# AI-Unicamp/interspeech_ser

Measured on AMD Instinct MI355X. Metric: utterances/sec (10 s @16 kHz) WavLM-large embed extract, higher is better.
Workload: dtype bf16; 1 GPU; microsoft/wavlm-large embed extract, batch=16 x 10 s @16 kHz per GPU, all 25 hidden states to HBM, mode=bf16; a counted step = 8 such batches (128 utterances per GPU), 2 in flight at a time; batch=16, batches_in_flight=2, frames_per_utt=499, parallelism=utterance-sharded x1, no collective (one process)

## Files before the change

include/ser_hip.h:

```cpp
#ifndef SER_HIP_H
#define SER_HIP_H

#include <stddef.h>
#include <stdint.h>

#ifdef __cplusplus
extern "C" {
#endif

#define SER_ABI_VERSION 18

#define SER_MODE_BF16  1
#define SER_MODE_FP32X 2
#define SER_MODE_FP16  3
#define SER_MODE_FP16X 4
#define SER_MODE_FP16Q 5

#define SER_MODE_FP16M 6

#define SER_ACT_NONE 0
#define SER_ACT_GELU 1

int         ser_version(void);
const char* ser_last_error(void);
// ... 174 lines not shown
typedef struct ser_row_center_args {
    const float* x; int64_t ldx; void* out_act; int64_t ldo_act; int64_t out_plane_stride;
    float* stats; float* shift; int32_t stat_groups, mode, rows, D;
    uint32_t* out_scale; int64_t out_scale_ld;
    uint32_t* range_flag;
} ser_row_center_args;
int ser_row_center_v(const ser_row_center_args* args, void* stream);

typedef struct ser_logmel_args {
    const float* wav; const int64_t* sample_offs; const float* mel; float* out; void* work; int32_t B, n_mels;
} ser_logmel_args;

typedef struct ser_pack_act_args {
    const float* x; void* out; int64_t ldo; int64_t out_plane_stride; int32_t B, C, T, halo, mode, reserved0;
    uint32_t* range_flag;
} ser_pack_act_args;
int ser_pack_act_v(const ser_pack_act_args* args, void* stream);

typedef struct ser_wave_frames_args {
    const float* wav; const int64_t* sample_offs; const int32_t* frame_offs; int32_t B, k, stride, mode;
    void* out; int64_t out_plane_stride; void* work; int32_t total_rows;
    int32_t no_norm;
    uint32_t* range_flag;
} ser_wave_frames_args;
int ser_wave_frames_v(const ser_wave_frames_args* args, void* stream);

#define SER_RESAMPLE_TILE 1024
typedef struct ser_resample_args {
    const float* wav; const int64_t* in_offs; const int64_t* out_offs;
    const int32_t* up; const int32_t* down; const int32_t* half; const int64_t* bank_off;
    const double* bank; float* out;
    int64_t total_in, total_out, max_out;
    int32_t B, reserved0;
} ser_resample_args;
int ser_resample_v(const ser_resample_args* args, void* stream);

typedef struct ser_gn_stats_args {
    const float* wav; const int64_t* sample_offs; const int32_t* frame_offs;
    const float* w; const float* bias; const float* gamma; const float* beta;
    const void* wave_stats;
    float* scale; float* shift; float* stat_out; void* work;
    int32_t B, C, k, stride, ld, no_norm;
    float eps; int32_t reserved0;
} ser_gn_stats_args;
int ser_gn_stats_v(const ser_gn_stats_args* args, void* stream);

// ... 310 lines not shown
```

interspeech_ser_amd/_lib.py:

```python
from __future__ import annotations

import ctypes as C
import os

import torch

_HERE = os.path.dirname(os.path.abspath(__file__))
LIB_PATH = os.environ.get("SER_HIP_LIB") or os.path.join(_HERE, "lib", "libserhip.so")

MODE_BF16 = 1
MODE_FP32X = 2
MODE_FP16 = 3
MODE_FP16X = 4
MODE_FP16Q = 5
MODE_FP16M = 6
ACT_NONE = 0
ACT_GELU = 1
WS_LOGMEL = 1
WS_WAVE_FRAMES = 2
WS_GN_STATS = 3
GRU_ERR_TIMEOUT = 1
RESAMPLE_TILE = 1024
SELECT_ROWS_TILE = 8
ABI_VERSION = 18
# ... 39 lines not shown
        ("gate_x", c_void_p), ("gate_x_ld", c_i64), ("gate_x_plane_stride", c_i64),
        ("gate_stat", c_void_p), ("gate_w", c_void_p), ("gate_cb", c_void_p),
        ("gate_x_planes", C.c_int32), ("reserved1", C.c_int32), ("gate_w_plane_stride", c_i64),
        ("out_scale", c_void_p), ("out_scale_ld", c_i64),
    ]


class LayerNormArgs(C.Structure):
    _fields_ = [
        ("x", c_void_p), ("ldx", c_i64), ("g", c_void_p), ("b", c_void_p), ("eps", c_float), ("gelu", C.c_int32),
        ("out_f32", c_void_p), ("ldo_f32", c_i64), ("out_act", c_void_p), ("ldo_act", c_i64), ("out_plane_stride", c_i64),
        ("mode", C.c_int32), ("rows", C.c_int32), ("D", C.c_int32), ("reserved0", C.c_int32),
        ("range_flag", c_void_p),
    ]


class WaveFramesArgs(C.Structure):
    _fields_ = [
        ("wav", c_void_p), ("sample_offs", c_void_p), ("frame_offs", c_void_p),
        ("B", C.c_int32), ("k", C.c_int32), ("stride", C.c_int32), ("mode", C.c_int32),
        ("out", c_void_p), ("out_plane_stride", c_i64), ("work", c_void_p),
        ("total_rows", C.c_int32), ("no_norm", C.c_int32),
        ("range_flag", c_void_p),
    ]


class GnStatsArgs(C.Structure):
    _fields_ = [
        ("wav", c_void_p), ("sample_offs", c_void_p), ("frame_offs", c_void_p),
        ("w", c_void_p), ("bias", c_void_p), ("gamma", c_void_p), ("beta", c_void_p),
        ("wave_stats", c_void_p),
        ("scale", c_void_p), ("shift", c_void_p), ("stat_out", c_void_p), ("work", c_void_p),
        ("B", C.c_int32), ("C", C.c_int32), ("k", C.c_int32), ("stride", C.c_int32), ("ld", C.c_int32), ("no_norm", C.c_int32),
        ("eps", c_float), ("reserved0", C.c_int32),
    ]


class RowCenterArgs(C.Structure):
    _fields_ = [
        ("x", c_void_p), ("ldx", c_i64), ("out_act", c_void_p), ("ldo_act", c_i64), ("out_plane_stride", c_i64),
        ("stats", c_void_p), ("shift", c_void_p),
        ("stat_groups", C.c_int32), ("mode", C.c_int32), ("rows", C.c_int32), ("D", C.c_int32),
        ("out_scale", c_void_p), ("out_scale_ld", c_i64), ("range_flag", c_void_p),
    ]


# ... 369 lines not shown
```

interspeech_ser_amd/csrc/gemm.hip:

```cpp
#include "ser_common.h"
#include "launch_plan.h"
#ifndef SER_GEMM_PP
#define SER_GEMM_PP 27
#endif
#include <stdlib.h>
#include <stdio.h>
#include <utility>
#ifdef SER_GEMM_DBG
extern "C" { void* ser_gemm_dbg_ptr = nullptr; }
__device__ unsigned long long* ser_gemm_dbg_dev = nullptr;
#endif

typedef const __attribute__((address_space(1))) void* gptr_t;
typedef __attribute__((address_space(3))) void* lptr_t;

__device__ __forceinline__ const char* uniform_ptr(const void* p) {
    const uint64_t v = (uint64_t)p;
    const uint32_t lo = __builtin_amdgcn_readfirstlane((uint32_t)v), hi = __builtin_amdgcn_readfirstlane((uint32_t)(v >> 32));
    return (const char*)(((uint64_t)hi << 32) | lo);
}
template <int BYTES>
__device__ __forceinline__ void dma_lds(const void* ubase, uint32_t voff, uint32_t lds_addr) {
    static_assert(BYTES == 16 || BYTES == 4, "dwordx4 or dword");
    if constexpr (BYTES == 16)
// ... 19 lines not shown
    else static_assert(N < 0, "add a case");
}

__device__ __forceinline__ void mfma_scale8(f32x4& acc, const i32x8& a, const i32x8& b, int sa, int sb) {
    asm volatile("v_mfma_scale_f32_16x16x128_f8f6f4 %0, %1, %2, %0, %3, %4 op_sel_hi:[0,0,0]" : "+v"(acc) : "v"(a), "v"(b), "v"(sa), "v"(sb));
}
__device__ __forceinline__ void mfma_scale_drain() {
    asm volatile("s_nop 15\n\ts_nop 15\n\ts_nop 7" ::: "memory");
}

template <int WM, int WN, int TM, int TN, int BK, int ST, int MODE, bool LNEPI, int OM = MODE>
__global__ __launch_bounds__(64 * WM * WN, 2)
void ser_gemm_kernel(const ser_gemm_args p) {
    constexpr int NW = WM * WN, NT = 64 * NW;
    constexpr int BM = WM * TM * 16, BN = WN * TN * 16;
    constexpr int CH = BK / 8;
    constexpr int ROWB = BK * 2;
    constexpr int RPP = 1024 / ROWB;
    constexpr bool M16 = (MODE == SER_MODE_FP16M);
    constexpr int NPL = M16 ? 1 : mode_traits<MODE>::planes;
    constexpr int A_BYTES = BM * ROWB, W_BYTES = BN * ROWB, STAGE = NPL * (A_BYTES + W_BYTES);
    static_assert(!M16 || (BK == 64 && !LNEPI && (BM + BN) % 64 == 0), "FP16M: 64-deep K tiles, dense epilogue");
    constexpr int SCW = BM + BN;
    constexpr int LA = BM / RPP / NW, LW = BN / RPP / NW;
    constexpr int LPT = NPL * (LA + LW);
    constexpr int KS = BK / 32;
    static_assert(BM % (RPP * NW) == 0 && BN % (RPP * NW) == 0, "tile/wave mismatch");
    extern __shared__ __attribute__((aligned(16))) char lds[];

    const int tid = threadIdx.x;
    const int lane = tid & 63;
    const int wave = __builtin_amdgcn_readfirstlane(tid >> 6);
    const int wm = wave / WN, wn = wave % WN;
#ifdef SER_GEMM_DBG
    const unsigned long long dbg_e0 = __builtin_amdgcn_s_memtime();
#endif

    const int ntn = (p.N + BN - 1) / BN;
    const int ntm = (p.M + BM - 1) / BM;
    int bid = blockIdx.x;
    {
        const int nwg = ntm * ntn;
        const int q = nwg >> 3, r = nwg & 7, xcd = bid & 7;
        const int base = (xcd < r) ? xcd * (q + 1) : r * (q + 1) + (xcd - r) * q;
        bid = base + (bid >> 3);
    }
    const int mt = bid / ntn;
    const int nt = bid - mt * ntn;
    const int g = blockIdx.y;
    const int m0 = mt * BM, n0 = nt * BN;
// ... 43 lines not shown
        int i = sc_is_a ? m0 + r : n0 + r - BM;
        const int lim = sc_is_a ? p.M : p.N;
        i = i < lim ? i : lim - 1;
        sc_off = (uint32_t)i * 4u;
    }
    int i_kk = 0, i_cc = 0, i_cj = 0, i_stage = 0;
    const char* is_ua = nullptr; const char* is_uw = nullptr;
    uint32_t is_dstA = 0, is_dstW = 0;
    auto issue_begin = [&]() {
        int64_t koffA = (int64_t)i_cj * p.ldj + (int64_t)i_cc * BK;
        int64_t koffW = (int64_t)i_kk * BK;
        if constexpr (M16) {
            koffA = (int64_t)(i_kk >> 1) * BK + (i_kk & 1) * p.a_plane_stride;
            koffW = (int64_t)(i_kk >> 1) * BK + (i_kk & 1) * p.w_plane_stride;
            if (i_kk & 1) dma_lds<4>(sc_base + (int64_t)(i_kk >> 1) * sc_step, sc_off, lds0 + (uint32_t)(ST * STAGE + (LNEPI ? 0 : BM * 8) + (i_stage * SCW + sc_chunk * 64) * 4));
        }
        is_dstA = lds0 + i_stage * STAGE + wave * 1024;
        is_dstW = is_dstA + NPL * A_BYTES;
        is_ua = Atile + koffA * 2;
        is_uw = Wtile + koffW * 2;
    };
    auto issue_piece = [&](int j) {
        const int pl = j / (LA + LW), q = j % (LA + LW);
        if (q < LA) dma_lds<16>(is_ua + (int64_t)pl * p.a_plane_stride * 2, aoff[q < LA ? q : 0], is_dstA + pl * A_BYTES + q * NW * 1024);
        else dma_lds<16>(is_uw + (int64_t)pl * p.w_plane_stride * 2, woff[q >= LA ? q - LA : 0], is_dstW + pl * W_BYTES + (q - LA) * NW * 1024);
    };
    auto issue_end = [&]() {
        ++i_kk; ++i_cc;
        if (i_cc == tpc) { i_cc = 0; ++i_cj; }
        i_stage = (i_stage + 1 == ST) ? 0 : i_stage + 1;
    };
    auto issue = [&]() {
        issue_begin();
#pragma unroll
        for (int j = 0; j < LPT; ++j) issue_piece(j);
        issue_end();
    };

    f32x4 acc[TN][TM];
#pragma unroll
    for (int a = 0; a < TN; ++a)
#pragma unroll
        for (int b = 0; b < TM; ++b) acc[a][b] = (f32x4){0.f, 0.f, 0.f, 0.f};

    const int frow = lane & 15, fq = lane >> 4;
    const int fsw = (BK == 64) ? (lane & 7) : ((frow >> 1) & 3);
    int offA[KS], offW[KS];
// ... 681 lines not shown
```

interspeech_ser_amd/csrc/launch_plan.h:

```cpp
#pragma once
#include <stddef.h>
#include <stdint.h>
#include <stdio.h>
#include <stdlib.h>
#include "../../include/ser_hip.h"

int ser_fail(int code, const char* fmt, ...);

#ifdef SER_EXPERIMENTS
static inline long ser_knob(const char* name, long dflt) { const char* e = getenv(name); return e ? atol(e) : dflt; }
#else
constexpr long ser_knob(const char*, long dflt) { return dflt; }
#endif

struct gemm_tile {
    const char* name;
    int WM, WN, TM, TN, BK, ST;
    bool LNEPI, two_plane;
    constexpr int BM() const { return WM * TM * 16; }
    constexpr int BN() const { return WN * TN * 16; }
    constexpr int threads() const { return 64 * WM * WN; }
    constexpr bool dense() const { return !LNEPI && BN() >= 128; }
};
enum gemm_tile_id {
    GEMM_128x128, GEMM_256x128, GEMM_256x256,
    GEMM_128x64, GEMM_LN512, GEMM_LN512_M64, GEMM_LN512_M32,
    GEMM_X_128x128x64, GEMM_X_256x128x32, GEMM_X_256x256x32, GEMM_X_128x64x32, GEMM_X_LN128x512x32,
    GEMM_TILES
};
constexpr gemm_tile GEMM_TILE[GEMM_TILES] = {
    {"128x128",         2, 2, 4, 4, 64, 2, false, false},
    {"256x128",         4, 2, 4, 4, 64, 3, false, false},
    {"256x256",         2, 4, 8, 4, 64, 2, false, false},
    {"128x64",          4, 1, 2, 4, 64, 2, false, false},
    {"LN512",           2, 4, 4, 8, 64, 2, true,  false},
    {"LN512_M64",       1, 8, 4, 4, 64, 2, true,  false},
    {"LN512_M32",       1, 4, 2, 8, 64, 2, true,  false},
    {"X_128x128x64",    4, 2, 2, 4, 64, 2, false, true},
    {"X_256x128x32",    4, 2, 4, 4, 32, 3, false, true},
    {"X_256x256x32",    4, 2, 4, 8, 32, 2, false, true},
    {"X_128x64x32",     4, 1, 2, 4, 32, 2, false, true},
    {"X_LN128x512x32",  2, 4, 4, 8, 32, 2, true,  true},
};

struct gemm_pair { int mode, om; };
constexpr gemm_pair GEMM_PAIR[] = {
    {SER_MODE_BF16, SER_MODE_BF16},
    {SER_MODE_FP16, SER_MODE_FP16},
    {SER_MODE_FP16, SER_MODE_FP16X},
    {SER_MODE_FP16M, SER_MODE_FP16M},
    {SER_MODE_FP16M, SER_MODE_FP16X},
    {SER_MODE_FP32X, SER_MODE_FP32X},
    {SER_MODE_FP32X, SER_MODE_FP16},
    {SER_MODE_FP16X, SER_MODE_FP16X},
    {SER_MODE_FP16X, SER_MODE_FP16},
    {SER_MODE_FP16X, SER_MODE_FP16M},
};
constexpr int GEMM_PAIRS = (int)(sizeof(GEMM_PAIR) / sizeof(GEMM_PAIR[0]));
constexpr int gemm_pair_index(int mode, int om) {
    for (int i = 0; i < GEMM_PAIRS; ++i)
        if (GEMM_PAIR[i].mode == mode && GEMM_PAIR[i].om == om) return i;
    return -1;
}
constexpr bool gemm_two_plane(int mode) { return mode == SER_MODE_FP32X || mode == SER_MODE_FP16X; }
constexpr bool gemm_tile_serves(const gemm_tile& t, gemm_pair p) {
    if (t.two_plane != gemm_two_plane(p.mode)) return false;
    if (p.mode == SER_MODE_FP16M) return t.dense() && t.BK == 64;
    if (p.om == p.mode) return true;
    if (t.two_plane && p.om == SER_MODE_FP16) return !t.LNEPI;
    return t.dense();
}

struct gemm_knobs {
    int ln_bm, n64, deepk;
    long t256_min, x32_256_min, x32_sq_min, m16_sq_min, m16_256_min;
};
static inline const gemm_knobs& gemm_knobs_get() {
    static const gemm_knobs k = {
        (int)ser_knob("SER_GEMM_LN_BM", 0), (int)ser_knob("SER_GEMM_N64", 1), (int)ser_knob("SER_GEMM_DEEPK_256x128", 1),
        ser_knob("SER_GEMM_T256_MIN", 150),
        ser_knob("SER_GEMM_X32_256_MIN", 100),
        ser_knob("SER_GEMM_X32_SQ_MIN", 150), ser_knob("SER_GEMM_M16_SQ_MIN", 100), ser_knob("SER_GEMM_M16_256_MIN", 100)};
    return k;
}

#ifdef SER_EXPERIMENTS
static inline int gemm_forced_tile(const ser_gemm_args* a) {
    struct Rule { int n, k, cfg; };
    static Rule rules[8];
    static const int nrules = [] {
        const char* e = getenv("SER_GEMM_FORCE");
        int n = 0;
        while (e && *e && n < 8) {
            int a0, a1, a2, used = 0;
            if (sscanf(e, "%d:%d:%d%n", &a0, &a1, &a2, &used) != 3) break;
            rules[n++] = {a0, a1, a2};
            e += used;
            if (*e == ',') ++e;
        }
        return n;
    }();
    for (int i = 0; i < nrules; ++i)
        if (rules[i].n == a->N && rules[i].k == a->K && rules[i].cfg >= 0 && rules[i].cfg <= GEMM_256x256) return rules[i].cfg;
    return -1;
}
#endif

static inline int gemm_pick_tile(const ser_gemm_args* a) {
    const gemm_knobs& kn = gemm_knobs_get();
    const long rt256 = (a->M + 255) / 256;
    const long t256sq = rt256 * ((a->N + 255) / 256) * a->groups;
    const long t256x128 = rt256 * ((a->N + 127) / 128) * a->groups;
    if (gemm_two_plane(a->mode)) {
        if (a->ln_gamma) return GEMM_X_LN128x512x32;
        if (kn.n64 && a->N <= 64) return GEMM_X_128x64x32;
        const long sq_rounds = (t256sq + 255) / 256;
        const bool sq_full = t256sq * 100 >= sq_rounds * 256 * 85;
        if (kn.x32_sq_min > 0 && a->N >= 256 && t256sq >= kn.x32_sq_min && sq_full && a->act == SER_ACT_NONE) return GEMM_X_256x256x32;
        if (kn.x32_256_min > 0 && a->N >= 128 && t256x128 >= kn.x32_256_min) return GEMM_X_256x128x32;
        return GEMM_X_128x128x64;
    }
    if (a->mode == SER_MODE_FP16M) {
        if (a->tile_cfg == 3 || (!a->tile_cfg && a->N >= 256 && t256sq >= kn.m16_sq_min)) return GEMM_256x256;
        if (a->tile_cfg == 2 || (!a->tile_cfg && a->N >= 128 && t256x128 >= kn.m16_256_min)) return GEMM_256x128;
        return GEMM_128x128;
    }
    if (a->ln_gamma) {
        const int bm = kn.ln_bm ? kn.ln_bm : (a->M >= 200 * 128 ? 128 : (a->M >= 200 * 64 ? 64 : 32));
        return bm == 128 ? GEMM_LN512 : (bm == 64 ? GEMM_LN512_M64 : GEMM_LN512_M32);
    }
    if (a->tile_cfg > 0) return a->tile_cfg - 1;
#ifdef SER_EXPERIMENTS
    if (const int forced = gemm_forced_tile(a); forced >= 0) return forced;
#endif
    if (a->N >= 256 && t256sq >= kn.t256_min) return GEMM_256x256;
    if (kn.n64 && a->N <= 64) return GEMM_128x64;
    if (kn.deepk && a->groups == 1 && a->K >= 2048 && a->N >= 128 && a->M >= 512) return GEMM_256x128;
    return GEMM_128x128;
}

struct gemm_launch {
    int tile, pair;
    unsigned grid_x, grid_y;
    int block, lds;
};

static inline int gemm_plan(const ser_gemm_args* a, gemm_launch* out) {
    if (!a || !a->A || !a->W) return ser_fail(-1, "ser_gemm: null operand");
    if (a->M <= 0 || a->N <= 0 || a->K <= 0) return ser_fail(-2, "ser_gemm: bad shape M=%d N=%d K=%d", a->M, a->N, a->K);
    if (a->K % 64) return ser_fail(-3, "ser_gemm: K=%d must be a multiple of 64", a->K);
    if (a->kc && (a->kc % 64 || a->K % a->kc)) return ser_fail(-4, "ser_gemm: kc=%d must divide K and be a multiple of 64", a->kc);
    if (a->N % 8) return ser_fail(-5, "ser_gemm: N=%d must be a multiple of 8", a->N);
    if (gemm_pair_index(a->mode, a->mode) < 0) return ser_fail(-6, "ser_gemm: bad mode %d", a->mode);
    if (a->mode == SER_MODE_FP16M) {
        if (!a->a_scale || !a->w_scale || a->a_scale_ld < a->M || a->w_scale_ld < a->N)
            return ser_fail(-23, "ser_gemm: FP16M needs a_scale / w_scale with *_scale_ld >= the row count");
        if (a->a_rowoff || a->kc || a->groups != 1 || a->ln_gamma || (a->lda % 64))
            return ser_fail(-23, "ser_gemm: FP16M takes plain row-major operands (no row map / conv chunks / groups / LayerNorm epilogue), lda %% 64 == 0");
    }
    if (a->out_mode == SER_MODE_FP16M || (a->mode == SER_MODE_FP16M && !a->out_mode && a->out_act)) {
        if (!a->out_scale || (a->N % 64) || (a->ldo_act % 64) || a->groups != 1 || a->ln_gamma)
            return ser_fail(-24, "ser_gemm: an FP16M out_act needs out_scale, N %% 64 == 0, ldo_act %% 64 == 0, groups == 1, no LayerNorm epilogue");
    }
    if (!a->a_rowoff && (a->lda % 8)) return ser_fail(-7, "ser_gemm: lda must be a multiple of 8");
    if (a->groups < 1) return ser_fail(-8, "ser_gemm: groups=%d", a->groups);
    if (!a->out_f32 && !a->out_act) return ser_fail(-9, "ser_gemm: no output");
    if ((a->ldo_f32 % 4) || (a->ldo_act % 4) || (a->ldr % 4) || (a->c_group_stride % 4))
        return ser_fail(-10, "ser_gemm: output/residual pitches must be multiples of 4");
    if (a->ln_gamma) {
        if (!a->ln_beta) return ser_fail(-11, "ser_gemm: ln_gamma without ln_beta");
        if (a->N > 512 || a->groups != 1 || a->residual)
            return ser_fail(-12, "ser_gemm: the LayerNorm epilogue needs N <= 512, groups == 1, no residual");
    }
    if (a->ln_stats_in) {
        if (!a->ln_colsum || a->ln_groups < 2 || a->ln_groups > 32 || (a->ln_groups & 1) || a->ln_gamma)
            return ser_fail(-14, "ser_gemm: deferred LayerNorm needs ln_colsum, an even ln_groups in [2,32] and no fused-LN epilogue");
    }
    if (a->stat_out && (a->ln_gamma || a->stat_groups < a->groups * ((a->N + 63) / 64)))
        return ser_fail(-15, "ser_gemm: stat_out needs stat_groups >= groups*ceil(N/64) and no fused-LN epilogue");
    if (a->shift_out && (!a->stat_out || a->ln_gamma)) return ser_fail(-19, "ser_gemm: shift_out needs stat_out and no fused-LN epilogue");
    if (a->mean_out && !a->ln_stats_in) return ser_fail(-20, "ser_gemm: mean_out needs ln_stats_in");
    if (a->lnstat_out && !a->ln_stats_in) return ser_fail(-20, "ser_gemm: lnstat_out needs ln_stats_in");
    const int om = a->out_mode ? a->out_mode : a->mode;
    const int pair = gemm_pair_index(a->mode, om);
    if (om != a->mode && !a->ln_gamma && pair < 0)
        return ser_fail(-21, "ser_gemm: out_mode %d with mode %d (FP32X -> FP16, FP16 <-> FP16X, FP16X <-> FP16M convert)", a->out_mode, a->mode);
    if (om != a->mode && a->ln_gamma) return ser_fail(-21, "ser_gemm: out_mode %d with the LayerNorm epilogue", a->out_mode);
    if (a->col_scale_end % 4) return ser_fail(-17, "ser_gemm: col_scale_end must be a multiple of 4");
    if (a->gn_scale && (!a->gn_shift || !a->gn_row_offs || a->gn_B < 1 || a->gn_ld < a->N || (a->gn_ld % 4) || a->groups != 1 ||
                        a->ln_gamma || a->ln_stats_in))
        return ser_fail(-25, "ser_gemm: gn_scale needs gn_shift, gn_row_offs, gn_B >= 1, gn_ld >= N (multiple of 4), groups == 1, "
                             "no LayerNorm epilogue and no deferred LayerNorm");
    if ((a->ldo_act % 8) || (a->c_group_stride % 8)) return ser_fail(-18, "ser_gemm: act pitch / group stride must be multiples of 8");
    if (a->f32_col_begin < 0 || (a->f32_col_begin % 8)) return ser_fail(-16, "ser_gemm: f32_col_begin must be a non-negative multiple of 8");
    if (a->tile_cfg < 0 || a->tile_cfg > 3) return ser_fail(-13, "ser_gemm: tile_cfg=%d (0 auto, 1..3)", a->tile_cfg);

    const int tile = gemm_pick_tile(a);
    const gemm_tile& t = GEMM_TILE[tile];
    if (!gemm_tile_serves(t, GEMM_PAIR[pair])) {
        if (a->mode == SER_MODE_FP16M) return ser_fail(-22, "ser_gemm: FP16M needs a dense tile (N > 64, no LayerNorm epilogue)");
        if (a->mode == SER_MODE_FP16X) return ser_fail(-22, "ser_gemm: FP16X -> FP16M output needs a dense tile (N > 64)");
        return ser_fail(-22, "ser_gemm: FP16 -> FP16X output needs a dense tile (N > 64, no LayerNorm epilogue)");
    }
    const int BM = t.BM(), BN = t.BN();
    out->tile = tile;
    out->pair = pair;
    out->grid_x = (unsigned)(((a->M + BM - 1) / BM) * ((a->N + BN - 1) / BN));
    out->grid_y = (unsigned)a->groups;
    out->block = t.threads();
    out->lds = (gemm_two_plane(a->mode) ? 2 : 1) * t.ST * (BM + BN) * t.BK * 2 + (t.LNEPI ? 0 : BM * 8)
             + (a->mode == SER_MODE_FP16M ? t.ST * (BM + BN) * 4 : 0);
    return 0;
}

constexpr int ATTN_BKV = 64;
constexpr int ATTN_NWV = 4;

struct attn_launch {
    int dhp, mode;
    bool pre, tbl, b2d, gb, occ;
    int nbuf, bias_stride;
    size_t lds;
    int nq;
    unsigned grid;
};
constexpr int attn_qk_planes(int mode) { return (mode == SER_MODE_FP32X || mode == SER_MODE_FP16X || mode == SER_MODE_FP16Q) ? 2 : 1; }
constexpr int attn_v_planes(int mode) { return (mode == SER_MODE_FP32X || mode == SER_MODE_FP16X) ? 2 : 1; }
constexpr bool attn_form_built(int dhp, int mode, bool pre, bool tbl, bool b2d, bool gb, bool occ) {
    if (b2d) return dhp == 64 && pre && !tbl && !gb && !occ && (mode == SER_MODE_BF16 || mode == SER_MODE_FP32X || mode == SER_MODE_FP16X);
    if (gb) return dhp == 64 && pre && tbl && !occ;
    if (occ) return dhp == 64 && attn_qk_planes(mode) == 1;
    return pre || (mode != SER_MODE_FP16X && mode != SER_MODE_FP16Q);
}
// ... 64 lines not shown
```

interspeech_ser_amd/csrc/rowops.hip:

```cpp
#include "row_common.h"

__global__ __launch_bounds__(1024) void wave_norm_kernel(const float* __restrict__ wav,
                                                         const int64_t* __restrict__ offs, float* __restrict__ out) {
    __shared__ double red[16];
    __shared__ float stat[2];
    const int b = blockIdx.x;
    const int64_t s0 = offs[b], n = offs[b + 1] - s0;
    const float* x = wav + s0;
    float* y = out + s0;
    const int tid = threadIdx.x, lane = tid & 63, wv = tid >> 6;

    double acc = 0.0;
    for (int64_t i = tid; i < n; i += 1024) acc += (double)x[i];
    for (int o = 32; o > 0; o >>= 1) acc += __shfl_xor(acc, o, 64);
    if (lane == 0) red[wv] = acc;
    __syncthreads();
    if (tid == 0) {
        double t = 0.0;
        for (int i = 0; i < 16; ++i) t += red[i];
        stat[0] = (float)(t / (double)n);
    }
    __syncthreads();
    const float mean = stat[0];
    acc = 0.0;
// ... 20 lines not shown

__global__ __launch_bounds__(256) void wave_stats_kernel(const float* __restrict__ wav, const int64_t* __restrict__ offs,
                                                         double* __restrict__ part ) {
    __shared__ double red[2][4];
    const int b = blockIdx.y, chunk = blockIdx.x;
    const int64_t s0 = offs[b], n = offs[b + 1] - s0;
    const int64_t per = (n + 63) / 64;
    const int64_t lo = chunk * per, hi = (lo + per < n) ? lo + per : n;
    double a1 = 0.0, a2 = 0.0;
    for (int64_t i = lo + threadIdx.x; i < hi; i += 256) { const double x = (double)wav[s0 + i]; a1 += x; a2 += x * x; }
    for (int o = 32; o > 0; o >>= 1) { a1 += __shfl_xor(a1, o, 64); a2 += __shfl_xor(a2, o, 64); }
    if ((threadIdx.x & 63) == 0) { red[0][threadIdx.x >> 6] = a1; red[1][threadIdx.x >> 6] = a2; }
    __syncthreads();
    if (threadIdx.x == 0) {
        part[((int64_t)b * 64 + chunk) * 2] = (red[0][0] + red[0][1]) + (red[0][2] + red[0][3]);
        part[((int64_t)b * 64 + chunk) * 2 + 1] = (red[1][0] + red[1][1]) + (red[1][2] + red[1][3]);
    }
}

template <int MODE>
__global__ __launch_bounds__(256) void wave_frames_kernel(const float* __restrict__ wav, const int64_t* __restrict__ soffs,
                                                          const int32_t* __restrict__ foffs, const double* __restrict__ part,
                                                          unsigned short* __restrict__ out, int64_t plane, int k, int stride, uint32_t* __restrict__ rflag,
                                                          int no_norm) {
    __shared__ float stat[2];
    float ramax = 0.f;
    const int b = blockIdx.y, tid = threadIdx.x;
    const int64_t s0 = soffs[b], n = soffs[b + 1] - s0;
    if (tid < 64) {
        double a1 = part[((int64_t)b * 64 + tid) * 2], a2 = part[((int64_t)b * 64 + tid) * 2 + 1];
        for (int o = 32; o > 0; o >>= 1) { a1 += __shfl_xor(a1, o, 64); a2 += __shfl_xor(a2, o, 64); }
        if (tid == 0) {
            const double mean = a1 / (double)n;
            const double var = a2 / (double)n - mean * mean;
            stat[0] = (float)mean;
            stat[1] = 1.0f / sqrtf((float)(var > 0.0 ? var : 0.0) + 1e-7f);
        }
    }
    __syncthreads();
    const float mean = no_norm ? 0.f : stat[0], rstd = no_norm ? 1.f : stat[1];
    const int row_begin = foffs[b], T = foffs[b + 1] - row_begin;
    const float* x = wav + s0;
    const int c = tid & 7;
    for (int t = blockIdx.x * 32 + (tid >> 3); t < T; t += gridDim.x * 32) {
        float v[8];
#pragma unroll
        for (int i = 0; i < 8; ++i) {
            const int j = c * 8 + i;
            v[i] = (j < k) ? (x[(int64_t)t * stride + j] - mean) * rstd : 0.f;
        }
        unsigned short* dst = out + (int64_t)(row_begin + t) * 64 + c * 8;
        store_act4<MODE>(dst, plane, v[0], v[1], v[2], v[3]);
        store_act4<MODE>(dst + 4, plane, v[4], v[5], v[6], v[7]);
        if constexpr (mode_traits<MODE>::f16) {
#pragma unroll
            for (int i = 0; i < 8; ++i) ramax = range_fold(ramax, v[i]);
        }
    }
    if constexpr (mode_traits<MODE>::f16) range_report(rflag, ramax);
}

extern "C" int ser_wave_frames_v(const ser_wave_frames_args* a, void* stream) {
    if (!a) return ser_fail(-1, "ser_wave_frames: null pointer");
    const float* wav = a->wav; const int64_t* sample_offs = a->sample_offs; const int32_t* frame_offs = a->frame_offs;
    const int B = a->B, k = a->k, stride = a->stride, mode = a->mode, total_rows = a->total_rows;
    void* out = a->out; const int64_t out_plane_stride = a->out_plane_stride; void* work = a->work;
    if (!wav || !sample_offs || !frame_offs || !out || !work) return ser_fail(-1, "ser_wave_frames: null pointer");
    if (B <= 0 || k < 1 || k > 64 || stride < 1 || total_rows <= 0) return ser_fail(-2, "ser_wave_frames: bad B/k/stride/rows");
    if (mode != SER_MODE_BF16 && mode != SER_MODE_FP32X && mode != SER_MODE_FP16X) return ser_fail(-3, "ser_wave_frames: bad mode");
    hipStream_t s = (hipStream_t)stream;
    hipLaunchKernelGGL(wave_stats_kernel, dim3(64, B), dim3(256), 0, s, wav, sample_offs, (double*)work);
    int blocks = ((total_rows + B - 1) / B + 31) / 32;
    if (blocks > 1024) blocks = 1024;
    if (blocks < 1) blocks = 1;
    ser_with_mode<SER_MODE_BF16, SER_MODE_FP32X, SER_MODE_FP16X>(mode, [&](auto M) {
        hipLaunchKernelGGL(wave_frames_kernel<M()>, dim3(blocks, B), dim3(256), 0, s, wav, sample_offs, frame_offs, (const double*)work,
                           (unsigned short*)out, out_plane_stride, k, stride, a->range_flag, a->no_norm);
    });
    return ser_check_launch("ser_wave_frames");
}

extern "C" int ser_wave_frames(const float* wav, const int64_t* sample_offs, const int32_t* frame_offs, int B, int k,
                               int stride, void* out, int64_t out_plane_stride, int mode, void* work, int total_rows,
                               void* stream) {
    ser_wave_frames_args a = {};
    a.wav = wav; a.sample_offs = sample_offs; a.frame_offs = frame_offs; a.B = B; a.k = k; a.stride = stride; a.mode = mode;
    a.out = out; a.out_plane_stride = out_plane_stride; a.work = work; a.total_rows = total_rows;
    return ser_wave_frames_v(&a, stream);
}

template <int CPL, int KT, int MODE>
__global__ __launch_bounds__(256) void conv0_kernel(const float* __restrict__ x, const int64_t* __restrict__ soffs,
                                                    const int32_t* __restrict__ foffs,
                                                    const float* __restrict__ w, const float* __restrict__ bias,
                                                    const float* __restrict__ lg, const float* __restrict__ lb,
                                                    unsigned short* __restrict__ out, int64_t plane,
                                                    int k, int stride, int rpg) {
    constexpr int C = CPL * 64;
    const int lane = threadIdx.x & 63;
    const int b = blockIdx.y;
// ... 730 lines not shown
```

interspeech_ser_amd/engine.py:

```python
from __future__ import annotations

import copy
import ctypes as C
import math
from dataclasses import dataclass
from typing import Dict, List, Optional, Sequence

import numpy as np
import torch

from . import _lib
from ._lib import check, lib
from .weights import check_f16_weight
from .config import EncoderGeometry, FAMILY_DATA2VEC_AUDIO, FAMILY_ROBERTA, FAMILY_W2V_BERT, FAMILY_WAVLM, FAMILY_WHISPER

MODES = {"bf16": _lib.MODE_BF16, "fp32x": _lib.MODE_FP32X, "f16": _lib.MODE_FP16, "f16q": _lib.MODE_FP16, "f16a": _lib.MODE_FP16,
         "f16x": _lib.MODE_FP16X, "f16m": _lib.MODE_FP16M, "f16mf": _lib.MODE_FP16M}
POST_LN_MODES = ("f16x", "fp32x", "bf16")
_PLANES = {_lib.MODE_BF16: 1, _lib.MODE_FP32X: 2, _lib.MODE_FP16: 1, _lib.MODE_FP16X: 2, _lib.MODE_FP16M: 2}
_DTYPE = {_lib.MODE_BF16: torch.bfloat16, _lib.MODE_FP32X: torch.bfloat16, _lib.MODE_FP16: torch.float16,
          _lib.MODE_FP16X: torch.float16, _lib.MODE_FP16M: torch.float16}
_PRODUCTS = {_lib.MODE_BF16: 1, _lib.MODE_FP32X: 3, _lib.MODE_FP16: 1, _lib.MODE_FP16X: 3, _lib.MODE_FP16M: 2}


import os as _os
_NO_SHIFT = _os.environ.get("SER_NO_SHIFT", "0") == "1"
_STEM_F16X = _os.environ.get("SER_STEM_F16X", "1") == "1"


def _ptr(t: Optional[torch.Tensor]) -> Optional[int]:
    return None if t is None else t.data_ptr()


def _stream() -> int:
    return torch.cuda.current_stream().cuda_stream


class Sz(int):

    def __new__(cls, value: int, name: str):
        o = int.__new__(cls, value)
        o.name = name
        return o


class Tape:

    def __init__(self, capacity: int = 640):
        self.cmds = (_lib.Cmd * capacity)()
        self.n = 0
# ... 683 lines not shown
        super().__init__(geo, device, mode, post_ln=not geo.stable_layer_norm)
        if geo.family == FAMILY_WHISPER:
            raise ValueError("use WhisperEncoder for the whisper family")
        self.normalize = bool(normalize)
        self.gn_stem = geo.feat_extract_norm == "group"
        if (geo.family == FAMILY_DATA2VEC_AUDIO) != (geo.pos_conv_norm == "layer"):
            raise NotImplementedError("the LayerNorm'd positional conv stack is data2vec-audio's, and data2vec-audio has only that one")
        if geo.family == FAMILY_DATA2VEC_AUDIO:
            if self.gn_stem or not self.post_ln:
                raise NotImplementedError("data2vec-audio: the layer-norm conv stem with a post-LN encoder is the only form")
        elif self.post_ln != self.gn_stem:
            raise NotImplementedError("GroupNorm stems come with post-LN encoders and layer-norm stems with stable-LN ones")
        if not geo.feat_proj_layer_norm:
            raise NotImplementedError("feat_proj_layer_norm=False checkpoints are not supported")
        sd = state_dict
        D, C0 = geo.hidden, geo.conv_dim[0]
        if any(c != C0 for c in geo.conv_dim):
            raise NotImplementedError("conv_dim must be uniform")
        p0 = "feature_extractor.conv_layers.0"
        self.conv0_w = self._dev_f32(sd[p0 + ".conv.weight"].reshape(C0, geo.conv_kernel[0]))
        self.conv0_b = self._dev_f32(sd[p0 + ".conv.bias"]) if geo.conv_bias else None
        if geo.conv_kernel[0] > 64:
            raise NotImplementedError("conv layer 0 kernel wider than 64 taps")
        w0 = torch.zeros((C0, 64), dtype=torch.float32)
        w0[:, : geo.conv_kernel[0]] = sd[p0 + ".conv.weight"].reshape(C0, geo.conv_kernel[0]).float()
        self.conv0 = self._linear(w0, sd[p0 + ".conv.bias"] if geo.conv_bias else None, stem=True, name=p0 + ".conv.weight")
        if self.gn_stem:
            self.gn0 = self._ln_pair(sd, p0 + ".layer_norm")
            self.conv_ln = [None] * len(geo.conv_dim)
        else:
            self.conv_ln = [self._ln_pair(sd, f"feature_extractor.conv_layers.{i}.layer_norm") for i in range(len(geo.conv_dim))]
        self.convs: List[Linear] = []
        for i in range(1, len(geo.conv_dim)):
            p = f"feature_extractor.conv_layers.{i}.conv"
            w = sd[p + ".weight"].float()
            w2 = w.permute(0, 2, 1).reshape(w.shape[0], -1)
            self.convs.append(self._linear(w2, sd[p + ".bias"] if geo.conv_bias else None, stem=True, name=p + ".weight"))
        self.proj_ln = self._ln_pair(sd, "feature_projection.layer_norm")
        self.proj = self._linear(sd["feature_projection.projection.weight"], sd["feature_projection.projection.bias"], stem=True,
                                 name="feature_projection.projection.weight")
        G, k = geo.pos_conv_groups, geo.pos_conv_kernel
        Cg = D // G
        self.pos_cg, self.pos_kc = Cg, ((Cg + 63) // 64) * 64

        def pos_weight(w: torch.Tensor) -> torch.Tensor:
            wp = torch.zeros((G, Cg, k, self.pos_kc), dtype=torch.float32)
            wp[:, :, :, :Cg] = w.float().view(G, Cg, Cg, k).permute(0, 1, 3, 2)
# ... 14 lines not shown
                a = p + ".attention"
                self.layers.append(self._post_ln_layer_weights(
                    sd, a + ".q_proj", a + ".k_proj", a + ".v_proj", a + ".out_proj", p + ".layer_norm",
                    p + ".feed_forward.intermediate_dense", p + ".feed_forward.output_dense", p + ".final_layer_norm",
                    gate=self._gate_cols(sd, a) if geo.family == FAMILY_WAVLM else None))
                continue
            self.layers.append(self._layer_weights(
                sd, p, p + ".attention", p + ".layer_norm", p + ".final_layer_norm",
                p + ".feed_forward.intermediate_dense", p + ".feed_forward.output_dense",
                k_bias=True, gate=(geo.family == FAMILY_WAVLM), index=i))
        if geo.family == FAMILY_WAVLM:
            self.rel_embed = self._dev_f32(sd["encoder.layers.0.attention.rel_attn_embed.weight"])

    def _arena(self, slot: int, need: Dict[str, int]):
        arenas = self.__dict__.setdefault("_arenas", {})
        ar = arenas.get(slot)
        if ar is not None and all(ar["cap"][k] >= v for k, v in need.items()):
            return ar
        cap = {k: max(int(v), ar["cap"][k] if ar else 0) for k, v in need.items()}
        geo, dev = self.geo, self.device
        C0, D = geo.conv_dim[0], geo.hidden
        nl = len(geo.conv_dim)
        ar = dict(cap=cap)
        ar["frames"] = self._new_act(cap["rows0"], 64, stem=True)
        ar["wave_work"] = torch.empty(lib.ser_workspace_bytes(_lib.WS_WAVE_FRAMES, cap["B"], 0, 0, 0, self.stem_mode),
                                      dtype=torch.uint8, device=dev)
        ar["conv_act"] = [self._new_act(cap["rows0"], C0, stem=True), self._new_act(cap["rows1"], C0, stem=True)]
        ar["conv_rowoff"] = [torch.empty(cap["rows1"], dtype=torch.int32, device=dev) for _ in range(1, nl)]
        ar["halo_rowmap"] = torch.empty(cap["M"], dtype=torch.int32, device=dev)
        ar["pos_rowoff"] = torch.empty(cap["M"], dtype=torch.int32, device=dev)
        ar["feat_f32"] = torch.empty((cap["M"], C0), dtype=torch.float32, device=dev)
        ar["feat_act"] = self._new_act(cap["M"], C0, stem=True)
        ar["proj_f32"] = torch.empty((cap["M"], D), dtype=torch.float32, device=dev)
        ar["halo_act"] = self._new_act(cap["halo"], D, zero=True, extra_rows=1, stem=self.pos_in_stem)
        ar["states"] = torch.empty((geo.num_layers + 1, cap["M"], D), dtype=torch.float32, device=dev)
        ar["first_groups"] = 2
        if self.gn_stem:
            ar["gn_scale"] = torch.empty((cap["B"], C0), dtype=torch.float32, device=dev)
            ar["gn_shift"] = torch.empty((cap["B"], C0), dtype=torch.float32, device=dev)
            ar["gn_work"] = torch.empty(lib.ser_workspace_bytes(_lib.WS_GN_STATS, cap["B"], 0, 0, 0, self.stem_mode), dtype=torch.uint8, device=dev)
        if self.post_ln:
            self._post_ln_buffers(ar, cap["M"], 3 * D + (self._gate_width() if geo.family == FAMILY_WAVLM else 0))
        else:
            self._layer_buffers(ar, cap["M"], ar["first_groups"])
        if geo.family == FAMILY_WAVLM:
            ar["table"] = torch.empty(geo.heads * (2 * cap["Tmax"] - 1), dtype=torch.float32, device=dev)
        ar["tab_region"] = cap["B"] + 2
# ... 181 lines not shown
    def download(self, t: torch.Tensor) -> torch.Tensor:
        host = torch.empty(t.shape, dtype=t.dtype).pin_memory()
        host.copy_(t, non_blocking=True)
        torch.cuda.current_stream().synchronize()
        return host

    use_tape = True

    @_on_stream
    def forward(self, packed_wave: torch.Tensor, lengths: Sequence[int], slot: int = 0,
                last_state: Optional[int] = None) -> HiddenStates:
        pl = self._plan(lengths, slot)
        return self._launch_or_replay(self._arenas[slot], pl, packed_wave, self._check_last_state(last_state))

    def _launches(self, pl, packed_wave: torch.Tensor, last_state: Optional[int] = None) -> None:
        geo = self.geo
        B, M, D, C0 = pl["B"], pl["M"], geo.hidden, geo.conv_dim[0]
        self._wave_frames(pl, packed_wave)
        a_in = pl["conv_act"][0]
        if self.gn_stem:
            self._groupnorm_stem(pl, packed_wave)
        else:
            self._gemm(pl["frames"], self.conv0, pl["rows"][0], act=_lib.ACT_GELU, ln=self.conv_ln[0], ln_eps=1e-5, out_act=a_in,
                       k_algo=geo.conv_kernel[0], stem=True)
        nl = len(geo.conv_dim)
        for i in range(1, nl):
            rows = pl["rows"][i]
            if i < nl - 1:
                a_view = pl["conv_act"][i % 2].first_rows(rows)
                self._gemm(a_in, self.convs[i - 1], rows, a_rowoff=pl["conv_rowoff"][i - 1], act=_lib.ACT_GELU,
                           ln=self.conv_ln[i], ln_eps=1e-5, out_act=a_view, stem=True)
                a_in = a_view
            else:
                self._gemm(a_in, self.convs[i - 1], rows, a_rowoff=pl["conv_rowoff"][i - 1], act=_lib.ACT_GELU,
                           ln=self.conv_ln[i], ln_eps=1e-5, out_f32=pl["feat_f32"], ldo_f32=C0, stem=True)
        self._layernorm(pl["feat_f32"], C0, self.proj_ln, M, C0, out_act=pl["feat_act"], stem=True)
        self._gemm(pl["feat_act"], self.proj, M, out_f32=pl["proj_f32"], ldo_f32=D,
                   out_act=pl["halo_act"], out_rowmap=pl["halo_rowmap"], stem=True,
                   out_mode=self.stem_mode if self.pos_in_stem else self.mode)
        states = pl["states"]
        G, Cg, kc = geo.pos_conv_groups, self.pos_cg, self.pos_kc
        if geo.pos_conv_norm == "layer":
            self._pos_stack(pl, states)
            self._run_post_ln_layers(pl, states, B, pl["Tmax"], last_state)
            return
        self._gemm(pl["halo_act"], self.pos, M, a_rowoff=pl["pos_rowoff"], kc=kc, ldj=D, groups=G,
                   a_group_stride=Cg, w_group_stride=Cg * geo.pos_conv_kernel * kc, c_group_stride=Cg,
                   N=Cg, K=geo.pos_conv_kernel * kc, act=_lib.ACT_GELU, residual=pl["proj_f32"], ldr=D,
                   out_f32=pl["tmp"] if self.post_ln else states[0], ldo_f32=D, k_algo=geo.pos_conv_kernel * Cg, stem=self.pos_in_stem)
        if self.post_ln:
            self._layernorm(pl["tmp"], D, self.enc_ln, M, D, out_f32=states[0], out_act=pl["xa"])
            self._run_post_ln_layers(pl, states, B, pl["Tmax"], last_state)
            return
        self._run_layers(pl, states, pl["first_groups"], B, pl["Tmax"], last_state)

    def _wave_frames(self, pl, packed_wave: torch.Tensor) -> None:
        geo, fr = self.geo, pl["frames"]
        B, rows = pl["B"], pl["rows"][0]
        a = self._cmd("wave_frames")
        a.wav, a.sample_offs, a.frame_offs = packed_wave.data_ptr(), pl["sample_offs"].data_ptr(), pl["frame_offs0"].data_ptr()
        a.B, a.k, a.stride, a.mode = B, geo.conv_kernel[0], geo.conv_stride[0], self.stem_mode
        a.out, a.out_plane_stride, a.work, a.total_rows = fr.ptr, fr.plane_stride, pl["wave_work"].data_ptr(), rows
        a.no_norm = 0 if self.normalize else 1
        a.range_flag = self._flag
        self._issue(_lib.OP_WAVE_FRAMES, a, "ser_wave_frames", input="wav", B=B, total_rows=rows)

    def _pos_stack(self, pl, states) -> None:
        geo = self.geo
        M, D = pl["M"], geo.hidden
        G, Cg, kc, k = geo.pos_conv_groups, self.pos_cg, self.pos_kc, geo.pos_conv_kernel
        halo = pl["halo_act"]
        n = len(self.pos_stack)
        for j, lin in enumerate(self.pos_stack):
            self._gemm(halo, lin, M, a_rowoff=pl["pos_rowoff"], kc=kc, ldj=D, groups=G, a_group_stride=Cg, w_group_stride=Cg * k * kc,
                       c_group_stride=Cg, N=Cg, K=k * kc, out_f32=pl["tmp"], ldo_f32=D, k_algo=k * Cg, stem=self.pos_in_stem)
            if j + 1 < n:
                self._pos_ln(pl["tmp"], M, out_act=halo, rowmap=pl["halo_rowmap"], mode=self.stem_mode if self.pos_in_stem else self.mode)
            else:
                self._pos_ln(pl["tmp"], M, out_act=pl["xa"], mode=self.mode, residual=pl["proj_f32"], out_f32=states[0])

    def _pos_ln(self, x: torch.Tensor, rows: int, *, out_act: Optional[Act], mode: int, rowmap=None, residual=None, out_f32=None) -> None:
        D = self.geo.hidden
        last = residual is not None
        a = self._cmd("pos_ln")
        a.x, a.ldx = x.data_ptr(), D
        a.out_act = None if out_act is None else out_act.ptr
# ... 1711 lines not shown
```

Before: 2089 utterances/s.

## Add single-K-tile LayerNorm GEMM tiles for conv0 with 32-wide frame rows

Adds dedicated GEMM tile configs for the first conv layer, where K fits in a single K tile. They use a one-stage LDS allocation and a 1x4 wave layout that may only partially fill the A tile. The wave-frame packer gains a 32-wide row mode, so a 10-tap kernel is padded to 32 instead of 64 columns, halving frame bytes and conv0 MACs. Conv0 now defaults to the 32-deep BF16 variant, which adds new code paths and validation constraints.

```diff
diff --git a/include/ser_hip.h b/include/ser_hip.h
--- a/include/ser_hip.h
+++ b/include/ser_hip.h
@@ -220,6 +220,8 @@
     void* out; int64_t out_plane_stride; void* work; int32_t total_rows;
     int32_t no_norm;
     uint32_t* range_flag;
+    int32_t row_width;
+    int32_t reserved1;
 } ser_wave_frames_args;
 int ser_wave_frames_v(const ser_wave_frames_args* args, void* stream);
 
diff --git a/interspeech_ser_amd/_lib.py b/interspeech_ser_amd/_lib.py
--- a/interspeech_ser_amd/_lib.py
+++ b/interspeech_ser_amd/_lib.py
@@ -85,6 +85,7 @@
         ("out", c_void_p), ("out_plane_stride", c_i64), ("work", c_void_p),
         ("total_rows", C.c_int32), ("no_norm", C.c_int32),
         ("range_flag", c_void_p),
+        ("row_width", C.c_int32), ("reserved1", C.c_int32),
     ]
 
 
diff --git a/interspeech_ser_amd/csrc/gemm.hip b/interspeech_ser_amd/csrc/gemm.hip
--- a/interspeech_ser_amd/csrc/gemm.hip
+++ b/interspeech_ser_amd/csrc/gemm.hip
@@ -65,10 +65,13 @@
     constexpr int A_BYTES = BM * ROWB, W_BYTES = BN * ROWB, STAGE = NPL * (A_BYTES + W_BYTES);
     static_assert(!M16 || (BK == 64 && !LNEPI && (BM + BN) % 64 == 0), "FP16M: 64-deep K tiles, dense epilogue");
     constexpr int SCW = BM + BN;
-    constexpr int LA = BM / RPP / NW, LW = BN / RPP / NW;
+    constexpr int A_PIECES = BM / RPP;
+    constexpr bool A_PART = A_PIECES < NW;
+    constexpr int LA = A_PART ? 1 : BM / RPP / NW, LW = BN / RPP / NW;
     constexpr int LPT = NPL * (LA + LW);
     constexpr int KS = BK / 32;
-    static_assert(BM % (RPP * NW) == 0 && BN % (RPP * NW) == 0, "tile/wave mismatch");
+    static_assert((A_PART ? BM % RPP == 0 : BM % (RPP * NW) == 0) && BN % (RPP * NW) == 0, "tile/wave mismatch");
+    static_assert(!A_PART || (ST == 2 && NW == 4 && !M16), "a partial A fill needs the plain two-stage ring");
     extern __shared__ __attribute__((aligned(16))) char lds[];
 
     const int tid = threadIdx.x;
@@ -158,7 +161,7 @@
     };
     auto issue_piece = [&](int j) {
         const int pl = j / (LA + LW), q = j % (LA + LW);
-        if (q < LA) dma_lds<16>(is_ua + (int64_t)pl * p.a_plane_stride * 2, aoff[q < LA ? q : 0], is_dstA + pl * A_BYTES + q * NW * 1024);
+        if (q < LA) { if (!A_PART || wave < A_PIECES) dma_lds<16>(is_ua + (int64_t)pl * p.a_plane_stride * 2, aoff[q < LA ? q : 0], is_dstA + pl * A_BYTES + q * NW * 1024); }
         else dma_lds<16>(is_uw + (int64_t)pl * p.w_plane_stride * 2, woff[q >= LA ? q - LA : 0], is_dstW + pl * W_BYTES + (q - LA) * NW * 1024);
     };
     auto issue_end = [&]() {
diff --git a/interspeech_ser_amd/csrc/launch_plan.h b/interspeech_ser_amd/csrc/launch_plan.h
--- a/interspeech_ser_amd/csrc/launch_plan.h
+++ b/interspeech_ser_amd/csrc/launch_plan.h
@@ -17,6 +17,8 @@
     const char* name;
     int WM, WN, TM, TN, BK, ST;
     bool LNEPI, two_plane;
+    bool one_tile = false;
+    bool bf16_only = false;
     constexpr int BM() const { return WM * TM * 16; }
     constexpr int BN() const { return WN * TN * 16; }
     constexpr int threads() const { return 64 * WM * WN; }
@@ -26,8 +28,10 @@
     GEMM_128x128, GEMM_256x128, GEMM_256x256,
     GEMM_128x64, GEMM_LN512, GEMM_LN512_M64, GEMM_LN512_M32,
     GEMM_X_128x128x64, GEMM_X_256x128x32, GEMM_X_256x256x32, GEMM_X_128x64x32, GEMM_X_LN128x512x32,
+    GEMM_LN512_1S_M64, GEMM_LN512_1S_M64_K32, GEMM_LN512_1S_M32, GEMM_LN512_1S_M32_K32,
     GEMM_TILES
 };
+constexpr int GEMM_TILE_CFG_1S = 10;
 constexpr gemm_tile GEMM_TILE[GEMM_TILES] = {
     {"128x128",         2, 2, 4, 4, 64, 2, false, false},
     {"256x128",         4, 2, 4, 4, 64, 3, false, false},
@@ -41,6 +45,10 @@
     {"X_256x256x32",    4, 2, 4, 8, 32, 2, false, true},
     {"X_128x64x32",     4, 1, 2, 4, 32, 2, false, true},
     {"X_LN128x512x32",  2, 4, 4, 8, 32, 2, true,  true},
+    {"LN512_1S_M64",     1, 4, 4, 8, 64, 2, true, false, true, true},
+    {"LN512_1S_M64_K32", 1, 4, 4, 8, 32, 2, true, false, true, true},
+    {"LN512_1S_M32",     1, 4, 2, 8, 64, 2, true, false, true},
+    {"LN512_1S_M32_K32", 1, 4, 2, 8, 32, 2, true, false, true},
 };
 
 struct gemm_pair { int mode, om; };
@@ -65,6 +73,7 @@
 constexpr bool gemm_two_plane(int mode) { return mode == SER_MODE_FP32X || mode == SER_MODE_FP16X; }
 constexpr bool gemm_tile_serves(const gemm_tile& t, gemm_pair p) {
     if (t.two_plane != gemm_two_plane(p.mode)) return false;
+    if (t.bf16_only && p.mode != SER_MODE_BF16) return false;
     if (p.mode == SER_MODE_FP16M) return t.dense() && t.BK == 64;
     if (p.om == p.mode) return true;
     if (t.two_plane && p.om == SER_MODE_FP16) return !t.LNEPI;
@@ -107,6 +116,7 @@
 #endif
 
 static inline int gemm_pick_tile(const ser_gemm_args* a) {
+    if (a->tile_cfg >= GEMM_TILE_CFG_1S) return GEMM_LN512_1S_M64 + (a->tile_cfg - GEMM_TILE_CFG_1S);
     const gemm_knobs& kn = gemm_knobs_get();
     const long rt256 = (a->M + 255) / 256;
     const long t256sq = rt256 * ((a->N + 255) / 256) * a->groups;
@@ -148,7 +158,9 @@
 static inline int gemm_plan(const ser_gemm_args* a, gemm_launch* out) {
     if (!a || !a->A || !a->W) return ser_fail(-1, "ser_gemm: null operand");
     if (a->M <= 0 || a->N <= 0 || a->K <= 0) return ser_fail(-2, "ser_gemm: bad shape M=%d N=%d K=%d", a->M, a->N, a->K);
-    if (a->K % 64) return ser_fail(-3, "ser_gemm: K=%d must be a multiple of 64", a->K);
+    const bool one_stage = a->tile_cfg >= GEMM_TILE_CFG_1S && a->tile_cfg < GEMM_TILE_CFG_1S + (GEMM_TILES - GEMM_LN512_1S_M64);
+    const int k_unit = (one_stage && GEMM_TILE[GEMM_LN512_1S_M64 + (a->tile_cfg - GEMM_TILE_CFG_1S)].BK == 32) ? 32 : 64;
+    if (a->K % k_unit) return ser_fail(-3, "ser_gemm: K=%d must be a multiple of %d", a->K, k_unit);
     if (a->kc && (a->kc % 64 || a->K % a->kc)) return ser_fail(-4, "ser_gemm: kc=%d must divide K and be a multiple of 64", a->kc);
     if (a->N % 8) return ser_fail(-5, "ser_gemm: N=%d must be a multiple of 8", a->N);
     if (gemm_pair_index(a->mode, a->mode) < 0) return ser_fail(-6, "ser_gemm: bad mode %d", a->mode);
@@ -193,7 +205,14 @@
                              "no LayerNorm epilogue and no deferred LayerNorm");
     if ((a->ldo_act % 8) || (a->c_group_stride % 8)) return ser_fail(-18, "ser_gemm: act pitch / group stride must be multiples of 8");
     if (a->f32_col_begin < 0 || (a->f32_col_begin % 8)) return ser_fail(-16, "ser_gemm: f32_col_begin must be a non-negative multiple of 8");
-    if (a->tile_cfg < 0 || a->tile_cfg > 3) return ser_fail(-13, "ser_gemm: tile_cfg=%d (0 auto, 1..3)", a->tile_cfg);
+    if (a->tile_cfg < 0 || (a->tile_cfg > 3 && !one_stage)) return ser_fail(-13, "ser_gemm: tile_cfg=%d (0 auto, 1..3, 10..13)", a->tile_cfg);
+    if (one_stage) {
+        const gemm_tile& t1 = GEMM_TILE[GEMM_LN512_1S_M64 + (a->tile_cfg - GEMM_TILE_CFG_1S)];
+        const bool mode_ok = a->mode == SER_MODE_BF16 || (a->mode == SER_MODE_FP16 && !t1.bf16_only);
+        if (!a->ln_gamma || !mode_ok || a->K != k_unit || a->kc || a->a_rowoff)
+            return ser_fail(-13, "ser_gemm: tile_cfg=%d needs the LayerNorm epilogue, BF16%s, plain rows and exactly one K tile (K = %d)",
+                            a->tile_cfg, t1.bf16_only ? "" : " or FP16", k_unit);
+    }
 
     const int tile = gemm_pick_tile(a);
     const gemm_tile& t = GEMM_TILE[tile];
@@ -208,7 +227,8 @@
     out->grid_x = (unsigned)(((a->M + BM - 1) / BM) * ((a->N + BN - 1) / BN));
     out->grid_y = (unsigned)a->groups;
     out->block = t.threads();
-    out->lds = (gemm_two_plane(a->mode) ? 2 : 1) * t.ST * (BM + BN) * t.BK * 2 + (t.LNEPI ? 0 : BM * 8)
+    const int stages = t.one_tile ? 1 : t.ST;
+    out->lds = (gemm_two_plane(a->mode) ? 2 : 1) * stages * (BM + BN) * t.BK * 2 + (t.LNEPI ? 0 : BM * 8)
              + (a->mode == SER_MODE_FP16M ? t.ST * (BM + BN) * 4 : 0);
     return 0;
 }
diff --git a/interspeech_ser_amd/csrc/rowops.hip b/interspeech_ser_amd/csrc/rowops.hip
--- a/interspeech_ser_amd/csrc/rowops.hip
+++ b/interspeech_ser_amd/csrc/rowops.hip
@@ -66,7 +66,7 @@
 __global__ __launch_bounds__(256) void wave_frames_kernel(const float* __restrict__ wav, const int64_t* __restrict__ soffs,
                                                           const int32_t* __restrict__ foffs, const double* __restrict__ part,
                                                           unsigned short* __restrict__ out, int64_t plane, int k, int stride, uint32_t* __restrict__ rflag,
-                                                          int no_norm) {
+                                                          int no_norm, int wsh ) {
     __shared__ float stat[2];
     float ramax = 0.f;
     const int b = blockIdx.y, tid = threadIdx.x;
@@ -85,15 +85,16 @@
     const float mean = no_norm ? 0.f : stat[0], rstd = no_norm ? 1.f : stat[1];
     const int row_begin = foffs[b], T = foffs[b + 1] - row_begin;
     const float* x = wav + s0;
-    const int c = tid & 7;
-    for (int t = blockIdx.x * 32 + (tid >> 3); t < T; t += gridDim.x * 32) {
+    const int c = tid & ((1 << wsh) - 1);
+    const int rpb = 256 >> wsh;
+    for (int t = blockIdx.x * rpb + (tid >> wsh); t < T; t += gridDim.x * rpb) {
         float v[8];
 #pragma unroll
         for (int i = 0; i < 8; ++i) {
             const int j = c * 8 + i;
             v[i] = (j < k) ? (x[(int64_t)t * stride + j] - mean) * rstd : 0.f;
         }
-        unsigned short* dst = out + (int64_t)(row_begin + t) * 64 + c * 8;
+        unsigned short* dst = out + (((int64_t)(row_begin + t) << wsh) + c) * 8;
         store_act4<MODE>(dst, plane, v[0], v[1], v[2], v[3]);
         store_act4<MODE>(dst + 4, plane, v[4], v[5], v[6], v[7]);
         if constexpr (mode_traits<MODE>::f16) {
@@ -111,15 +112,18 @@
     void* out = a->out; const int64_t out_plane_stride = a->out_plane_stride; void* work = a->work;
     if (!wav || !sample_offs || !frame_offs || !out || !work) return ser_fail(-1, "ser_wave_frames: null pointer");
     if (B <= 0 || k < 1 || k > 64 || stride < 1 || total_rows <= 0) return ser_fail(-2, "ser_wave_frames: bad B/k/stride/rows");
+    const int width = a->row_width ? a->row_width : 64;
+    if ((width != 64 && width != 32) || k > width) return ser_fail(-4, "ser_wave_frames: row_width=%d (0 or 64, or 32 with k <= 32)", a->row_width);
     if (mode != SER_MODE_BF16 && mode != SER_MODE_FP32X && mode != SER_MODE_FP16X) return ser_fail(-3, "ser_wave_frames: bad mode");
     hipStream_t s = (hipStream_t)stream;
     hipLaunchKernelGGL(wave_stats_kernel, dim3(64, B), dim3(256), 0, s, wav, sample_offs, (double*)work);
-    int blocks = ((total_rows + B - 1) / B + 31) / 32;
+    const int rpb = width == 32 ? 64 : 32;
+    int blocks = ((total_rows + B - 1) / B + rpb - 1) / rpb;
     if (blocks > 1024) blocks = 1024;
     if (blocks < 1) blocks = 1;
     ser_with_mode<SER_MODE_BF16, SER_MODE_FP32X, SER_MODE_FP16X>(mode, [&](auto M) {
         hipLaunchKernelGGL(wave_frames_kernel<M()>, dim3(blocks, B), dim3(256), 0, s, wav, sample_offs, frame_offs, (const double*)work,
-                           (unsigned short*)out, out_plane_stride, k, stride, a->range_flag, a->no_norm);
+                           (unsigned short*)out, out_plane_stride, k, stride, a->range_flag, a->no_norm, width == 32 ? 2 : 3);
     });
     return ser_check_launch("ser_wave_frames");
 }
diff --git a/interspeech_ser_amd/engine.py b/interspeech_ser_amd/engine.py
--- a/interspeech_ser_amd/engine.py
+++ b/interspeech_ser_amd/engine.py
@@ -26,6 +26,7 @@
 import os as _os
 _NO_SHIFT = _os.environ.get("SER_NO_SHIFT", "0") == "1"
 _STEM_F16X = _os.environ.get("SER_STEM_F16X", "1") == "1"
+_CONV0_TILE_DEFAULT = 11
 
 
 def _ptr(t: Optional[torch.Tensor]) -> Optional[int]:
@@ -755,7 +756,17 @@
         self.conv0_b = self._dev_f32(sd[p0 + ".conv.bias"]) if geo.conv_bias else None
         if geo.conv_kernel[0] > 64:
             raise NotImplementedError("conv layer 0 kernel wider than 64 taps")
-        w0 = torch.zeros((C0, 64), dtype=torch.float32)
+        self.conv0_cfg = 0
+        if not self.gn_stem and self.stem_mode in (_lib.MODE_BF16, _lib.MODE_FP16) and C0 <= 512:
+            self.conv0_cfg = int(_os.environ.get("SER_GEMM_CONV0_TILE", _CONV0_TILE_DEFAULT))
+            if self.conv0_cfg not in (0, 10, 11, 12, 13):
+                raise ValueError(f"SER_GEMM_CONV0_TILE={self.conv0_cfg}: 0 or 10..13")
+            if self.conv0_cfg in (10, 11) and self.stem_mode == _lib.MODE_FP16:
+                self.conv0_cfg += 2
+            if self.conv0_cfg in (11, 13) and geo.conv_kernel[0] > 32:
+                self.conv0_cfg -= 1
+        self.conv0_k = 32 if self.conv0_cfg in (11, 13) else 64
+        w0 = torch.zeros((C0, self.conv0_k), dtype=torch.float32)
         w0[:, : geo.conv_kernel[0]] = sd[p0 + ".conv.weight"].reshape(C0, geo.conv_kernel[0]).float()
         self.conv0 = self._linear(w0, sd[p0 + ".conv.bias"] if geo.conv_bias else None, stem=True, name=p0 + ".conv.weight")
         if self.gn_stem:
@@ -816,7 +827,7 @@
         C0, D = geo.conv_dim[0], geo.hidden
         nl = len(geo.conv_dim)
         ar = dict(cap=cap)
-        ar["frames"] = self._new_act(cap["rows0"], 64, stem=True)
+        ar["frames"] = self._new_act(cap["rows0"], self.conv0_k, stem=True)
         ar["wave_work"] = torch.empty(lib.ser_workspace_bytes(_lib.WS_WAVE_FRAMES, cap["B"], 0, 0, 0, self.stem_mode),
                                       dtype=torch.uint8, device=dev)
         ar["conv_act"] = [self._new_act(cap["rows0"], C0, stem=True), self._new_act(cap["rows1"], C0, stem=True)]
@@ -1044,7 +1055,7 @@
             self._groupnorm_stem(pl, packed_wave)
         else:
             self._gemm(pl["frames"], self.conv0, pl["rows"][0], act=_lib.ACT_GELU, ln=self.conv_ln[0], ln_eps=1e-5, out_act=a_in,
-                       k_algo=geo.conv_kernel[0], stem=True)
+                       k_algo=geo.conv_kernel[0], stem=True, tile_cfg=self.conv0_cfg)
         nl = len(geo.conv_dim)
         for i in range(1, nl):
             rows = pl["rows"][i]
@@ -1084,6 +1095,7 @@
         a.B, a.k, a.stride, a.mode = B, geo.conv_kernel[0], geo.conv_stride[0], self.stem_mode
         a.out, a.out_plane_stride, a.work, a.total_rows = fr.ptr, fr.plane_stride, pl["wave_work"].data_ptr(), rows
         a.no_norm = 0 if self.normalize else 1
+        a.row_width = fr.cols
         a.range_flag = self._flag
         self._issue(_lib.OP_WAVE_FRAMES, a, "ser_wave_frames", input="wav", B=B, total_rows=rows)
 
```

After: 2097 utterances/s, median of 6. About the same (+0.4%).
